# gue-ni/raytracer.c

Measured on AMD Instinct MI355X. Metric: ray-bounces/sec, higher is better.
Workload: dtype f64

## Files before the change

### include/rt_hip.h

```cpp
#ifndef RT_HIP_H
#define RT_HIP_H

#include <stddef.h>
#include <stdint.h>

#ifdef __cplusplus
extern "C" {
#endif

#define RT_HIP_TILE 8
#define RT_HIP_TILE_PIXELS 64

enum
{
  RT_HIP_OK = 0,
  RT_HIP_ENODEV = -1,
  RT_HIP_EINVAL = -2,
  RT_HIP_ENOMEM = -3,
  RT_HIP_ERUNTIME = -4,
  RT_HIP_ELIMIT = -5,
  RT_HIP_ECANCELLED = -6,
};

typedef struct
// ... 409 lines not shown
int rt_hip_selftest_math(int op, const double *h_a, const double *h_b, double *h_out, size_t n, int device);

int rt_hip_selftest_intersect(int kind, const double *h_rays, const double *h_prims, size_t n, double near_R,
                              uint8_t *h_hit, double *h_tuv, uint64_t *h_keep, int device);

enum
{
  RT_HIP_FAIL_ALLOC_PARK_WS = 1,
  RT_HIP_FAIL_ALLOC_WIDE_PEND = 2,
  RT_HIP_FAIL_ALLOC_TAIL_WS = 4
};
void rt_hip_selftest_fail_alloc(uint32_t mask);

uint64_t rt_hip_mixed_grid_launches(void);

int rt_hip_selftest_pool_slots(int device, uint32_t *park_slots_per_xcd, uint32_t *pend_slots_per_xcd);

int rt_hip_selftest_xcc(uint32_t n_workgroups, uint32_t h_counts[16], int device);


void rt_hip_set_cancel_flag(const volatile int *flag);

int rt_hip_render_image(const RtHipSphere *spheres, size_t n_spheres, const RtHipMesh *meshes,
                        size_t n_meshes, const RtHipCamera *camera, const RtHipParams *params,
                        int n_devices, float *h_image_rgb, uint8_t *h_image_rgb8, uint64_t *h_stats,
                        double *kernel_seconds);

void rt_hip_release_cache(void);
uint64_t rt_hip_cache_builds(void);

// ... 20 lines not shown
```

### raytracer.c_amd/csrc/pt_body_pooled.h

```cpp
#ifndef PT_BODY_POOLED_H
#define PT_BODY_POOLED_H


#ifndef PT_MIN_WAVES
#define PT_MIN_WAVES 5
#endif
#ifndef PT_MIN_WAVES_TRI
#define PT_MIN_WAVES_TRI 5
#endif
#ifndef PT_MIN_WAVES_CHK
#define PT_MIN_WAVES_CHK 5
#endif
#ifndef PT_MESH_BATCH
#define PT_MESH_BATCH 32
#endif
#ifndef PT_MESH_MAX_WAIT
#define PT_MESH_MAX_WAIT 16
#endif
#ifndef PT_DIR_PARK
#define PT_DIR_PARK 1
#endif
#ifndef PT_DIR_ROUNDS
#define PT_DIR_ROUNDS 4
#endif
// ... 2 lines not shown
#endif
#ifndef PT_DIR_MIN_LANES
#define PT_DIR_MIN_LANES 1
#endif
struct MixedUnit
{
  uint32_t j, chunk, chunks;
};
__device__ __forceinline__ MixedUnit mixed_unit(const PtLaunch &L, const bool LIST)
{
  const uint32_t n_whole = LIST ? 0u : L.n_whole;
  if (blockIdx.x < n_whole)
    return {blockIdx.x, 0u, 1u};
  const uint32_t r = blockIdx.x - n_whole, n_chunked = launch_slots(L, LIST) - n_whole;
  return {n_whole + r % n_chunked, r / n_chunked, L.sample_chunks};
}

template <bool CHECKER, bool TRIS, bool FILT_LDS, bool GEOM_LDS, bool REFR = false, bool MIXED = false>
__device__ __forceinline__ void render_tiles_pooled(const PtLaunch &L, const bool LIST)
{
  static_assert(!MIXED || !REFR, "the mixed grid: fixed-point sums only");
  static_assert(!REFR || (CHECKER && FILT_LDS && (GEOM_LDS || !TRIS)), "the pooled refraction kernels: sphere scenes (staged, or streamed from memory) and small staged mesh scenes, every material");
  extern __shared__ __attribute__((aligned(16))) double lds[];
  __shared__ float out_f[PT_TILE_PIXELS * 3];
  __shared__ uint8_t out_b[PT_TILE_PIXELS * 3 + 64];
  __shared__ unsigned long long wg_stats[2];
  __shared__ double cam_lds[PT_CAM_LDS_DOUBLES];
  __shared__ unsigned long long pix_sum[REFR ? 1 : PT_TILE_PIXELS * 3];
  __shared__ unsigned long long pix_win[REFR ? PT_TILE_PIXELS * 3 * PT_WIN_N : 1];
  __shared__ unsigned long long pend_free[REFR ? PT_BLOCK / 64 : 1][2];
// ... 51 lines not shown
  if (threadIdx.x < 3)
    pix_nan[threadIdx.x] = 0;
  if (!REFR && threadIdx.x < PT_TILE_PIXELS * 3)
    pix_sum[threadIdx.x] = 0;
  if (REFR)
  {
    for (uint32_t k = threadIdx.x; k < PT_TILE_PIXELS * 3 * PT_WIN_N; k += PT_BLOCK)
      pix_win[k] = 0;
    if (threadIdx.x < 2 * (PT_BLOCK / 64))
      pend_free[threadIdx.x >> 1][threadIdx.x & 1u] = ~0ull;
    if (threadIdx.x == 0)
      pend_slot_lds = pt_pool_acquire(L.pend_flags, L.pend_slots_per_xcd, L.status, PT_FAIL_PEND_SLOT);
  }
  if (threadIdx.x < PT_TILE_PIXELS)
  {
    const uint32_t t0 = L.tile_first + launch_slot(L, MIXED ? mixed_unit(L, LIST).j : blockIdx.x % launch_slots(L, LIST), LIST) * L.tile_stride;
    const uint32_t kx = (t0 % L.tiles_x) * PT_TILE + (threadIdx.x & 7u), ky = (t0 / L.tiles_x) * PT_TILE + (threadIdx.x >> 3);
    pix_key[threadIdx.x] = rt_rng_pixel_key(L.seed, ky * (uint32_t)L.width + kx);
  }
  camera_to_lds(L, cam_lds);
  PHASE(9);
  __syncthreads();
  PHASE(10);

  const uint32_t wave = threadIdx.x >> 6;
  const uint32_t slot = launch_slot(L, MIXED ? mixed_unit(L, LIST).j : blockIdx.x % launch_slots(L, LIST), LIST);
  const uint32_t chunk = MIXED ? mixed_unit(L, LIST).chunk : blockIdx.x / launch_slots(L, LIST);
  const uint32_t tile = L.tile_first + slot * L.tile_stride;
  const bool cull_ok = S.n_sph + S.n_tri <= 64u * CULL_WORDS;
  if (mf_sized && threadIdx.x < PT_MFMA16_ROWS)
  {
    uint16_t row[16];
    if (!pt_mfma16_row(L.scene.entry_src + PT_ENTRY_SRC_STRIDE * (size_t)(mf_first + threadIdx.x), L.near_R, S.filt_shift, row))
      atomicOr(&mf_bad, 1u);
    const uint32_t m = mfma16_row_of(threadIdx.x);
#pragma unroll
    for (int h = 0; h < 2; h++)
      mf_a[32 * h + m] = u32x4_t{row[8 * h + 0] | ((uint32_t)row[8 * h + 1] << 16), row[8 * h + 2] | ((uint32_t)row[8 * h + 3] << 16),
                                 row[8 * h + 4] | ((uint32_t)row[8 * h + 5] << 16), row[8 * h + 6] | ((uint32_t)row[8 * h + 7] << 16)};
  }
  if (SWAP && FILT_LDS && cull_ok)
// ... 449 lines not shown
    }
    PHASE(4);
    if (!PARK)
      radiance_to_sums();
    P.Ls = {0, 0, 0};
    PHASE(5);
  }

  if (n_rays)
  {
    atomicAdd(&wg_stats[0], (unsigned long long)n_rays);
    atomicAdd(&wg_stats[1], (unsigned long long)n_casts);
  }
  __syncthreads();
  PHASE(12);

  if (REFR)
  {
    if (!pend_ok && threadIdx.x < 3)
      pix_nan[threadIdx.x] = ~0ull;
    __syncthreads();
    if (L.sample_chunks == 1 && !L.acc_keep)
    {
      if (threadIdx.x < PT_TILE_PIXELS * 3)
      {
        const uint32_t t = threadIdx.x / 3u, c = threadIdx.x - 3u * t;
        const bool inside = (tile % L.tiles_x) * PT_TILE + (t & 7u) < (uint32_t)L.width && (tile / L.tiles_x) * PT_TILE + (t >> 3) < (uint32_t)L.height;
        win_normalize(&pix_win[threadIdx.x * PT_WIN_N]);
        double mean = win_value(&pix_win[threadIdx.x * PT_WIN_N]) * (1.0 / (double)L.samples);
        mean = ((pix_nan[c] >> t) & 1ull) ? __longlong_as_double(0x7FF8000000000000ll) : mean;
// ... 12 lines not shown
        unsigned long long *const acc = L.acc_ws + ((size_t)slot * (PT_TILE_PIXELS * 3) + threadIdx.x) * PT_WIN_N;
#pragma unroll
        for (int k = 0; k < PT_WIN_N; k++)
          if (w[k] != 0ull)
            atomicAdd(&acc[k], w[k]);
      }
      if (threadIdx.x < 3 && pix_nan[threadIdx.x] != 0)
        atomicOr(&L.acc_ws[(size_t)L.tile_count * (PT_TILE_PIXELS * 3 * PT_WIN_N) + (size_t)slot * 3 + threadIdx.x], pix_nan[threadIdx.x]);
      store_tile(L, out_f, out_b, wg_stats, tile, slot, S.n_sph + S.n_tri, false, chunk == 0);
    }
    if (pend_ok && threadIdx.x == 0)
      atomicExch(&L.pend_flags[pend_slot], 0u);
  }
  else if (MIXED ? ((!LIST && blockIdx.x < L.n_whole) || L.sample_chunks == 1) && !L.acc_keep : L.sample_chunks == 1 && !L.acc_keep)
  {
    finish_pixels(L, pix_sum, pix_nan, tile, out_f, out_b);
    __syncthreads();
    store_tile(L, out_f, out_b, wg_stats, tile, slot, S.n_sph + S.n_tri, true, true);
    PHASE(13);
#ifdef PT_PHASE
    if ((threadIdx.x & 63u) == 0u && L.stats && (blockIdx.x & 31u) == 0u)
      for (int k = 0; k < PT_PHASE_SLOTS; k++)
        atomicAdd(&L.stats[64 + k], pt_phase_acc[threadIdx.x >> 6][k]);
#endif
  }
  else
  {
    const uint32_t n_whole = MIXED && !LIST ? L.n_whole : 0u;
    if (threadIdx.x < PT_TILE_PIXELS * 3 && pix_sum[threadIdx.x] != 0)
      atomicAdd(&L.acc_ws[(size_t)(slot - n_whole) * (PT_TILE_PIXELS * 3) + threadIdx.x], pix_sum[threadIdx.x]);
    if (threadIdx.x < 3 && pix_nan[threadIdx.x] != 0)
      atomicOr(&L.acc_ws[(size_t)(L.tile_count - n_whole) * (PT_TILE_PIXELS * 3) + (size_t)(slot - n_whole) * 3 + threadIdx.x], pix_nan[threadIdx.x]);
    store_tile(L, out_f, out_b, wg_stats, tile, slot, S.n_sph + S.n_tri, false, chunk == 0);
  }
#ifdef PT_PHASE
  if (threadIdx.x == 0 && L.stats && (L.diag_flags & 4u))
  {
    L.stats[80 + 2 * (size_t)blockIdx.x] = wg_began;
    L.stats[81 + 2 * (size_t)blockIdx.x] = wall_clock64();
  }
#endif
}

#endif
```

### raytracer.c_amd/csrc/pt_device.h

```cpp
#ifndef PT_DEVICE_H
#define PT_DEVICE_H

#include <math.h>
#include <stdint.h>

#define PT_TILE 8
#define PT_TILE_PIXELS 64
#define PT_SLICES 4
#define PT_BLOCK 256
#define PT_MAT_STRIDE 8
#define PT_FILT_LDS_MAX 256
#ifndef PT_BVH_LEAF
#define PT_BVH_LEAF 15
#endif
#define PT_BVH_NODE_WORDS 16
#define PT_BVH_SRC_DOUBLES 16
#ifndef PT_BVH_COUNT_BITS
#define PT_BVH_COUNT_BITS 4
#endif
#define PT_BVH_LEAF_FLAG 0x80000000u
#define PT_BVH_STACK 24
#define PT_GEOM_STRIDE 4
#define PT_FILT_STRIDE 6
#define PT_TRI32_STRIDE 16
// ... 258 lines not shown
  char *park_ws;
  uint32_t *park_flags;
  uint32_t park_slots_per_xcd;
  double *pend_ws;
  uint32_t *pend_flags;
  uint32_t pend_slots_per_xcd, pend_entries;
  uint64_t pend_slot_doubles;
  uint32_t *status;
  unsigned long long *acc_ws;
  float *tiles_rgb;
  uint8_t *tiles_rgb8;
  unsigned long long *stats;
  const uint32_t *slot_list;
  uint32_t slot_count;
  uint32_t n_whole;
};

struct PtAovOut
{
  float *albedo, *normal, *depth;
  uint32_t *object, *hits;
};

struct PtQuery
{
  const double *rays;
  const double *t_max;
  uint64_t n;
  uint32_t camera_uv, normalize;
  uint32_t *status;
// ... 128 lines not shown
};
struct PtPlan
{
  int kernel;
  uint32_t sample_chunks;
  bool mixed;
  bool windowed;
  bool queued;
  uint32_t pend_entries, pend_columns;
};
PtPlan pt_plan_launch(const PtSceneView &scene, const PtPlanAsk &ask);
hipError_t pt_launch_render(const PtLaunch &launch, hipStream_t stream, int which);
bool pt_kernel_takes_chunks(int which);
uint32_t pt_resident_workgroups(int which, const PtSceneView &scene);
hipError_t pt_launch_resolve(const PtLaunch &launch, const uint32_t *tile_samples, hipStream_t stream, int which);
hipError_t pt_launch_tile_error(const float *cur, const float *prev, int width, int height, uint32_t tile_first, uint32_t tile_stride,
                                uint32_t tile_count, float *error, hipStream_t stream);
hipError_t pt_launch_tile_freeze(const float *error, double threshold, int dilate, uint8_t *keep, uint32_t *tile_samples, int width,
                                 int height, uint32_t tile_first, uint32_t tile_stride, uint32_t tile_count, uint32_t done,
                                 uint32_t *slot_list, uint32_t *live_count, hipStream_t stream);
static inline uint32_t pt_pend_entries(const PtSceneView &scene, uint32_t integrator, int32_t max_depth)
{
  const bool two_children = integrator == 1u ? scene.any_mirror_glass != 0u : scene.any_refract != 0u;
  return two_children ? (uint32_t)max_depth + 2u : 1u;
}
const char *pt_kernel_name_of(int which);
int pt_kernel_count(void);
unsigned long long pt_kernel_launches(int which);
uint32_t pt_pool_slots_per_xcd(bool park_pool);
#ifdef PT_DEV_KERNELS
// ... 111 lines not shown
```

### raytracer.c_amd/csrc/pt_kernel.hip

```cpp
#include <hip/hip_runtime.h>
#include <stdint.h>
#include <stdlib.h>
#include <atomic>

#include "pt_device.h"
#include "rt_rng.h"

#include "pt_math.h"
#include "pt_intersect.h"
#include "pt_filter.h"
#include "pt_scene_ctx.h"
#include "pt_trace.h"
#include "pt_body_pooled.h"
#include "pt_body_queued.h"
#include "pt_body_static.h"

enum PtKernelProps : uint32_t
{
  PEND_POOL = 1u, QUEUED = 2u, STAGES_NONE = 4u, WIDE_PEND = 8u, CHUNKS = 16u, WINDOWED = 32u, MIXED = 64u
};

#ifndef PT_MIN_WAVES_QUEUED
#define PT_MIN_WAVES_QUEUED 4
#endif
// ... 493 lines not shown
    const bool inside = (tile % L.tiles_x) * PT_TILE + (t & 7u) < (uint32_t)L.width &&
                        (tile / L.tiles_x) * PT_TILE + (t >> 3) < (uint32_t)L.height;
    const double inv_s = 1.0 / (double)samples;
    double mean = ((double)(long long)sums[threadIdx.x] * L.acc_inv_scale) * inv_s;
    const double quiet_nan = __longlong_as_double(0x7FF8000000000000ll);
    mean = ((nan_mask[c] >> t) & 1ull) ? quiet_nan : mean;
    out_f[threadIdx.x] = inside ? (float)mean : 0.f;
    out_b[threadIdx.x] = inside ? tonemap(mean) : 0;
  }
}

extern "C" __global__ __launch_bounds__(PT_BLOCK) void pt_resolve_tiles(const PtLaunch L, const uint32_t *tile_samples)
{
  __shared__ float out_f[PT_TILE_PIXELS * 3];
  __shared__ uint8_t out_b[PT_TILE_PIXELS * 3 + 64];
  const uint32_t slot = L.n_whole + blockIdx.x;
  const int32_t samples = resolve_samples(L, tile_samples, slot);
  const uint32_t tile = L.tile_first + slot * L.tile_stride;
  if (L.acc_windows)
  {
    if (threadIdx.x < PT_TILE_PIXELS * 3)
    {
      const uint32_t t = threadIdx.x / 3u, c = threadIdx.x - 3u * t;
      const bool inside = (tile % L.tiles_x) * PT_TILE + (t & 7u) < (uint32_t)L.width && (tile / L.tiles_x) * PT_TILE + (t >> 3) < (uint32_t)L.height;
      unsigned long long w[PT_WIN_N];
#pragma unroll
      for (int k = 0; k < PT_WIN_N; k++)
        w[k] = L.acc_ws[((size_t)slot * (PT_TILE_PIXELS * 3) + threadIdx.x) * PT_WIN_N + k];
      win_normalize(w);
      double mean = win_value(w) * (1.0 / (double)samples);
      const unsigned long long nan_mask = L.acc_ws[(size_t)L.tile_count * (PT_TILE_PIXELS * 3 * PT_WIN_N) + (size_t)slot * 3 + c];
// ... 112 lines not shown
  part[threadIdx.x] = n;
  __syncthreads();
  for (uint32_t step = 1; step < PT_COMPACT_THREADS; step <<= 1)
  {
    const uint32_t add = threadIdx.x >= step ? part[threadIdx.x - step] : 0u;
    __syncthreads();
    part[threadIdx.x] += add;
    __syncthreads();
  }
  uint32_t at = part[threadIdx.x] - n;
  for (uint32_t k = k0; k < k1; k++)
    if (tile_samples[k] == 0u)
      slot_list[at++] = k;
  if (threadIdx.x == PT_COMPACT_THREADS - 1)
    *live_count = part[threadIdx.x];
}

extern "C" __global__ __launch_bounds__(256) void pt_selftest_math(int op, const double *a, const double *b,
                                                                  double *out, size_t n)
{
  __shared__ double tab[PT_ATAN_TAB];
  atan_table_to_lds(tab);
  __syncthreads();
  for (size_t i = (size_t)blockIdx.x * blockDim.x + threadIdx.x; i < n; i += (size_t)gridDim.x * blockDim.x)
  {
    double r = 0;
    if (op == 0)
      r = sqrt_unscaled(a[i]);
    else if (op == 1)
      r = div_small_int(a[i], b[i], 1.0 / b[i]);
// ... 580 lines not shown
  if (k.has(PEND_POOL) && (launch.pend_ws == nullptr || launch.pend_entries < pt_pend_entries(launch.scene, launch.integrator, launch.max_depth) ||
                      launch.pend_slot_doubles < (uint64_t)launch.pend_entries * PT_PEND_FIELDS_HOST * k.pend_columns()))
    return hipErrorInvalidValue;
  const bool queued = k.has(QUEUED);
  if (queued && (launch.park_ws == nullptr || launch.park_slots_per_xcd == 0u))
    return hipErrorInvalidValue;
  if (launch.sample_chunks > 1 && !k.has(CHUNKS))
    return hipErrorInvalidValue;
  if (queued)
    lds_bytes += (k.has(STAGES_NONE) ? (size_t)0 : (size_t)pt_filt_pair_slots(launch.scene.n_spheres) * 8u) +
                 (((size_t)max(launch.scene.bvh_depth, 1u) * PT_BLOCK * 3u + 15u) & ~(size_t)15u);
  if (launch.acc_keep && (k.has(CHUNKS) ? launch.acc_ws == nullptr || (launch.acc_windows != 0u) != k.has(WINDOWED) : launch.slice_ws == nullptr))
    return hipErrorInvalidValue;
  if (launch.n_whole != 0u && (!k.has(MIXED) || launch.n_whole >= launch.tile_count || launch.sample_chunks < 2u || launch.acc_keep || launch.slot_list))
    return hipErrorInvalidValue;
  const uint32_t n_chunked = launch.tile_count - launch.n_whole;
  if (launch.sample_chunks > 1 && !launch.acc_keep)
  {
    if ((launch.acc_windows != 0u) != k.has(WINDOWED) || launch.acc_ws == nullptr)
      return hipErrorInvalidValue;
    hipError_t e = hipMemsetAsync(launch.acc_ws, 0, (size_t)n_chunked * (k.has(WINDOWED) ? PT_ACC_WS_WORDS_WIN : PT_ACC_WS_WORDS) * sizeof(unsigned long long), stream);
    if (e != hipSuccess)
      return e;
  }
  if ((launch.slot_list != nullptr) != (launch.slot_count != 0u) || (launch.slot_list && !launch.acc_keep) || launch.slot_count > launch.tile_count)
    return hipErrorInvalidValue;
  const uint32_t n_units = launch.n_whole + (launch.slot_list ? launch.slot_count : n_chunked) * launch.sample_chunks;
  hipError_t e = launch_staged(kernel, queued ? (n_units + PT_BLOCK / 64 - 1) / (PT_BLOCK / 64) : n_units, lds_bytes, stream, launch);
  if (e == hipSuccess && launch.sample_chunks > 1 && !launch.acc_keep)
    e = launch_staged(pt_resolve_tiles, n_chunked, 0, stream, launch, static_cast<const uint32_t *>(nullptr));
// ... 45 lines not shown
  const uint32_t tiles_x = ((uint32_t)width + PT_TILE - 1) / PT_TILE, waves = PT_BLOCK / 64u;
  hipLaunchKernelGGL(pt_tile_error, dim3((tile_count + waves - 1u) / waves), dim3(PT_BLOCK), 0, stream, cur, prev, width, height, tiles_x,
                     tile_first, tile_stride, tile_count, error);
  return hipGetLastError();
}

hipError_t pt_launch_tile_freeze(const float *error, double threshold, int dilate, uint8_t *keep, uint32_t *tile_samples, int width,
                                 int height, uint32_t tile_first, uint32_t tile_stride, uint32_t tile_count, uint32_t done,
                                 uint32_t *slot_list, uint32_t *live_count, hipStream_t stream)
{
  const uint32_t tiles_x = ((uint32_t)width + PT_TILE - 1) / PT_TILE, tiles_y = ((uint32_t)height + PT_TILE - 1) / PT_TILE;
  if (error)
    hipLaunchKernelGGL(pt_tile_keep, dim3((tile_count + 255u) / 256u), dim3(256), 0, stream, error, tile_samples, tiles_x, tiles_y, tile_first,
                       tile_stride, tile_count, threshold, dilate, keep);
  hipLaunchKernelGGL(pt_tile_compact, dim3(1), dim3(PT_COMPACT_THREADS), 0, stream, keep, tile_samples, tile_count, done, slot_list, live_count);
  return hipGetLastError();
}

hipError_t pt_launch_selftest_intersect(int kind, const double *rays, const double *prims, const double *entry_src,
                                        float *filt, float *tri32, uint32_t n, double near_R, double filt_shift,
                                        uint8_t *hit, double *tuv, unsigned long long *keep, hipStream_t stream)
{
  if (n == 0)
    return hipSuccess;
  if (kind == 2 && (!PT_MFMA16 || n % 64u != 0u))
    return hipErrorNotSupported;
  hipLaunchKernelGGL(pt_build_filter, dim3(min(1024u, (n + 255u) / 256u)), dim3(256), 0, stream, entry_src, n, near_R, filt);
  if (kind == 2)
  {
    hipLaunchKernelGGL(pt_selftest_mfma16, dim3(n / 64u), dim3(64), 0, stream, rays, prims, entry_src, reinterpret_cast<const f32x2 *>(filt), n,
// ... 111 lines not shown
```

### raytracer.c_amd/csrc/rt_hip_shim.hip

```cpp
#include <hip/hip_runtime.h>
#include <rccl/rccl.h>

#include <algorithm>
#include <atomic>
#include <chrono>
#include <cmath>
#include <cstdarg>
#include <cstddef>
#include <cstdio>
#include <cstdlib>
#include <cstring>
#include <limits>
#include <mutex>
#include <new>
#include <utility>
#include <vector>

#include "pt_device.h"
#include "rt_hip.h"
#include "rt_rng.h"
#include "bvh_build.h"
#include "rt_staging.h"

static_assert(sizeof(RtHipSphere) == 88, "RtHipSphere must match the reference Object");
// ... 231 lines not shown

}

struct TableSet
{
  double near_R = 0;
  float *filt = nullptr, *bvh_nodes = nullptr;
  hipEvent_t built = nullptr;
  std::vector<std::pair<hipStream_t, hipEvent_t>> readers;
  uint64_t stamp = 0;
  int users = 0;
  bool owned = false;
};
#define RT_TABLE_SETS 8

struct RtHipScene
{
  int device = 0;
  PtSceneView view{};
  mutable std::mutex table_mutex;
  mutable std::vector<TableSet> tables;
  mutable uint64_t table_clock = 0;
  size_t filt_bytes = 0, bvh_nodes_bytes = 0;
  mutable char *park_ws = nullptr;
  mutable uint32_t park_slots_per_xcd = 0;
  mutable bool park_tried = false;
  void *blob = nullptr;
  double reach = 0;
  double max_emission = 0;
  bool any_mirror_glass = false;
  double max_center = 0;
  int n_big = 0;
  double big_r[8] = {0}, big_c[8] = {0};
// ... 74 lines not shown
  m[2] = color[1] * inv;
  m[3] = color[2] * inv;
  m[4] = emission[0];
  m[5] = emission[1];
  m[6] = emission[2];
  uint64_t bits = flags;
  memcpy(&m[7], &bits, sizeof bits);
}




std::atomic<uint32_t> g_fail_alloc{0};

thread_local int g_last_kernel = -1;

size_t pad256(size_t b) { return (b + 255) & ~(size_t)255; }

hipError_t table_set_wait(const TableSet &t)
{
  hipError_t first = t.built ? hipEventSynchronize(t.built) : hipSuccess;
  for (auto &r : t.readers)
    if (const hipError_t e = hipEventSynchronize(r.second); first == hipSuccess)
      first = e;
  return first;
}

void table_set_free(TableSet &t)
{
  for (auto &r : t.readers)
// ... 30 lines not shown
    for (const TableSet &t : scene->tables)
      if (t.users > 0)
        return fail(RT_HIP_EINVAL, "a launch of this scene is being submitted");
    return RT_HIP_OK;
  }
  int drain() const
  {
    for (const TableSet &t : scene->tables)
      HIP_TRY(table_set_wait(t));
    return RT_HIP_OK;
  }
  void stale() const
  {
    for (TableSet &t : scene->tables)
      t.near_R = -1.0;
  }
  int broke(hipError_t e, const char *what) const
  {
    (void)hipGetLastError();
    scene->unusable = true;
    return fail(RT_HIP_ERUNTIME, "%s: %s; the scene is unusable now (destroy it)", what, hipGetErrorString(e));
  }
};

int acquire_tables(const RtHipScene *scene, double near_R, hipStream_t stream, float **filt, float **bvh_nodes, size_t *slot)
{
  std::lock_guard<std::mutex> lock(scene->table_mutex);
  std::vector<TableSet> &tables = scene->tables;
  if (const int rc = scene_usable(scene, "a launch"))
    return rc;
// ... 349 lines not shown
    }
  {
    std::lock_guard<std::mutex> slock(g_status_mutex);
    for (int d = 0; d < 64; d++)
      if (g_status[d])
      {
        (void)hipSetDevice(d);
        (void)hipDeviceSynchronize();
        (void)hipFree(g_status[d]);
        g_status[d] = nullptr;
      }
  }
  (void)hipSetDevice(prev);
}

struct GridTailWs
{
  unsigned long long *ws = nullptr;
  size_t bytes = 0;
  hipEvent_t done = nullptr;
  hipStream_t stream = nullptr;
  bool used = false;
  uint32_t resident = 0;
  int resident_kernel = -1;
  size_t resident_lds = 0;
};
std::mutex g_tail_mutex;
GridTailWs g_tail[64];
std::atomic<uint64_t> g_mixed_launches{0};

constexpr uint32_t GRID_TAIL_MIN_ROUNDS = 8, GRID_TAIL_ROUNDS = 1, GRID_TAIL_CHUNKS = 4, GRID_TAIL_MIN_SAMPLES = 128;

bool grid_split_for(const PtLaunch &L, const PtPlan &plan, int device, uint32_t *n_whole, uint32_t *chunks)
{
  if (!plan.mixed || plan.sample_chunks != 1u || L.acc_keep || L.slot_list || L.tile_count < 2u || L.samples < 2)
    return false;
  const char *uni = getenv("RT_HIP_GRID_UNIFORM");
  if (uni && uni[0] == '1')
    return false;
  if (const char *e = getenv("RT_HIP_GRID_SPLIT"))
// ... 17 lines not shown
    if (t.resident_kernel != plan.kernel || t.resident_lds != lds)
    {
      t.resident = pt_resident_workgroups(plan.kernel, L.scene);
      t.resident_kernel = plan.kernel;
      t.resident_lds = lds;
    }
    resident = t.resident;
  }
  if (resident == 0u || (uint64_t)L.tile_count < (uint64_t)GRID_TAIL_MIN_ROUNDS * resident)
    return false;
  *n_whole = L.tile_count - GRID_TAIL_ROUNDS * resident;
  *chunks = GRID_TAIL_CHUNKS;
  return true;
}

unsigned long long *grid_tail_ws(int device, uint32_t n_chunked, hipStream_t stream)
{
  if (device < 0 || device >= 64 || (g_fail_alloc.load() & RT_HIP_FAIL_ALLOC_TAIL_WS))
    return nullptr;
  GridTailWs &t = g_tail[device];
  const size_t need = (size_t)n_chunked * PT_ACC_WS_WORDS * sizeof(unsigned long long);
  if (t.bytes < need)
  {
    if (t.ws)
    {
      if (hipDeviceSynchronize() != hipSuccess)
      {
        (void)hipGetLastError();
        return nullptr;
      }
      (void)hipFree(t.ws);
      t.ws = nullptr;
    }
    t.bytes = 0;
    t.used = false;
    if (hipMalloc(&t.ws, need) != hipSuccess)
    {
      (void)hipGetLastError();
      t.ws = nullptr;
      return nullptr;
    }
    t.bytes = need;
  }
  if (!t.done && hipEventCreateWithFlags(&t.done, hipEventDisableTiming) != hipSuccess)
  {
    (void)hipGetLastError();
    t.done = nullptr;
    return nullptr;
  }
  if (t.used && t.stream != stream && hipStreamWaitEvent(stream, t.done, 0) != hipSuccess)
  {
    (void)hipGetLastError();
    return nullptr;
  }
  return t.ws;
}

void grid_tail_used(int device, hipStream_t stream)
{
  GridTailWs &t = g_tail[device];
  if (hipEventRecord(t.done, stream) != hipSuccess)
  {
    (void)hipGetLastError();
    (void)hipStreamSynchronize(stream);
    t.used = false;
    return;
  }
  t.stream = stream;
  t.used = true;
}

void grid_tail_release()
{
  std::lock_guard<std::mutex> lock(g_tail_mutex);
  int prev = 0;
  (void)hipGetDevice(&prev);
  for (int d = 0; d < 64; d++)
    if (g_tail[d].ws || g_tail[d].done)
    {
      (void)hipSetDevice(d);
      (void)hipDeviceSynchronize();
      if (g_tail[d].done)
        (void)hipEventDestroy(g_tail[d].done);
      if (g_tail[d].ws)
        (void)hipFree(g_tail[d].ws);
      g_tail[d] = GridTailWs();
    }
  (void)hipSetDevice(prev);
}

uint32_t tiles_x_of(int width) { return ((uint32_t)width + PT_TILE - 1) / PT_TILE; }
uint32_t tiles_y_of(int height) { return ((uint32_t)height + PT_TILE - 1) / PT_TILE; }

int check_params(const RtHipParams *p)
{
  if (!p)
    return fail(RT_HIP_EINVAL, "params is NULL");
  if (p->width < 2 || p->height < 2)
    return fail(RT_HIP_EINVAL, "width and height must be >= 2 (the reference divides by width-1, height-1)");
  if (p->samples < 1 || p->samples > (1 << 26))
// ... 3237 lines not shown
  v.n_bvh_nodes = c->n_triangles ? std::max(1u, c->n_triangles / 8u) : 0u;
  v.any_checker = c->any_checker ? 1u : 0u;
  v.any_refract = c->any_refract ? 1u : 0u;
  v.any_mirror_glass = c->any_mirror_glass ? 1u : 0u;
  v.wide_range = c->wide_range ? 1u : 0u;
  v.mesh_round = c->mesh_round ? 1u : 0u;
  const PtPlanAsk ask = {.integrator = c->integrator, .samples = c->samples_per_chunk, .max_depth = c->max_depth, .max_emission = c->max_emission,
                         .sample_chunks = 1, .have_park_ws = c->have_park_ws != 0, .wide_pend_ok = c->wide_pend_ok != 0};
  return pt_kernel_name_of(pt_plan_launch(v, ask).kernel);
}

void rt_hip_selftest_fail_alloc(uint32_t mask) { g_fail_alloc.store(mask); }

uint64_t rt_hip_mixed_grid_launches(void) { return g_mixed_launches.load(); }

int rt_hip_selftest_pool_slots(int device, uint32_t *park_slots_per_xcd, uint32_t *pend_slots_per_xcd)
{
  if (!have_device(device))
    return fail(RT_HIP_ENODEV, "no HIP device %d", device);
  DeviceScope scope(device);
  HIP_TRY(scope.status);
  if (park_slots_per_xcd)
    *park_slots_per_xcd = pt_pool_slots_per_xcd(true);
  if (pend_slots_per_xcd)
    *pend_slots_per_xcd = pt_pool_slots_per_xcd(false);
  return RT_HIP_OK;
}

int rt_hip_pool_bytes(int device, size_t *park_ws_bytes, size_t *pend_pool_bytes)
{
// ... 126 lines not shown
      rc = fail(RT_HIP_EINVAL, "tile_count x sample_chunks exceeds the grid limit");
    std::unique_lock<std::mutex> tail_lock(g_tail_mutex, std::defer_lock);
    uint32_t n_whole = 0, tail_chunks = 0;
    if (!rc && sample_chunks == 1 && !d_workspace && grid_split_for(L, plan, scene->device, &n_whole, &tail_chunks))
    {
      tail_lock.lock();
      if (unsigned long long *ws = grid_tail_ws(scene->device, L.tile_count - n_whole, st))
      {
        L.acc_ws = ws;
        L.n_whole = n_whole;
        L.sample_chunks = tail_chunks;
      }
      else
        tail_lock.unlock();
    }
    const hipError_t e = rc ? hipSuccess : pt_launch_render(L, st, plan.kernel);
    if (tail_lock.owns_lock())
    {
      grid_tail_used(scene->device, st);
      if (e == hipSuccess && L.n_whole != 0u)
        g_mixed_launches.fetch_add(1);
      tail_lock.unlock();
    }
    if (pend_lock.owns_lock())
      pend_lock.unlock();
    release_tables(scene, slot, st);
    if (!rc)
      rc = launched(e, pt_kernel_name_of(plan.kernel));
    if (!rc)
      g_last_kernel = plan.kernel;
    return rc;
  });
}


int rt_hip_accum_create(const RtHipScene *scene, const RtHipCamera *camera, const RtHipParams *params, RtHipAccum **out)
{
  if (out)
    *out = nullptr;
  if (!scene || !camera || !params || !out)
    return fail(RT_HIP_EINVAL, "scene, camera, params and out are required");
  if (params->samples < 1)
    return fail(RT_HIP_EINVAL, "the sample budget (params->samples) must be >= 1");
  return guarded("rt_hip_accum_create", [&]() -> int {
    PtLaunch L;
// ... 1031 lines not shown
```

### raytracer.c_amd/rt_amd/abi.py

```python
import ctypes as C
import os

PKG_DIR = os.path.dirname(os.path.dirname(os.path.abspath(__file__)))
REPO_ROOT = os.path.dirname(PKG_DIR)
SHIM_PATH = os.environ.get("RT_HIP_SHIM_PATH") or os.path.join(PKG_DIR, "csrc", "librt_hip.so")
HOST_PATH = os.path.join(PKG_DIR, "host", "libraytracer_amd.so")

M_DEFAULT, M_REFLECTION, M_REFRACTION, M_CHECKERED = 2, 4, 8, 16
TILE, TILE_PIXELS, TILE_FLOATS = 8, 64, 192
STAT_RAYS, STAT_CASTS, STAT_TESTS, STAT_SAMPLES, NSTATS = 0, 1, 2, 3, 4
FAIL_ALLOC_PARK_WS, FAIL_ALLOC_WIDE_PEND, FAIL_ALLOC_TAIL_WS = 1, 2, 4
FAIL_PEND_SLOT, FAIL_PARK_SLOT = 1, 2
EINVAL = -2
PASS_FN = C.CFUNCTYPE(None, C.c_int, C.c_int, C.c_double, C.c_void_p)


class Vec2(C.Structure):
    _fields_ = [("x", C.c_double), ("y", C.c_double)]


class Vec3(C.Structure):
    _fields_ = [("x", C.c_double), ("y", C.c_double), ("z", C.c_double)]

    def tuple(self):
# ... 229 lines not shown
    "rt_hip_untile": (C.c_int, [C.c_void_p, C.c_void_p, C.c_int32, C.c_int32, C.c_uint32, C.c_uint32, C.c_uint32,
                                C.c_void_p, C.c_void_p, C.c_void_p]),
    "rt_hip_set_cancel_flag": (None, [C.c_void_p]),
    "rt_hip_release_cache": (None, []),
    "rt_hip_cache_builds": (C.c_uint64, []),
    "rt_hip_set_device_map": (C.c_int, [C.POINTER(C.c_int), C.c_int]),
    "rt_hip_last_image_phases": (None, [C.POINTER(C.c_double)]),
    "rt_hip_pool_bytes": (C.c_int, [C.c_int, C.POINTER(C.c_size_t), C.POINTER(C.c_size_t)]),
    "rt_hip_last_launch_kernel": (C.c_char_p, []),
    "rt_hip_kernel_count": (C.c_int, []),
    "rt_hip_kernel_launches": (C.c_char_p, [C.c_int, C.POINTER(C.c_uint64)]),
    "rt_hip_kernel_for_class": (C.c_char_p, [C.c_void_p]),
    "rt_hip_launch_status": (C.c_int, [C.c_int, C.POINTER(C.c_uint32)]),
    "rt_hip_selftest_fail_alloc": (None, [C.c_uint32]),
    "rt_hip_mixed_grid_launches": (C.c_uint64, []),
    "rt_hip_selftest_pool_slots": (C.c_int, [C.c_int, C.POINTER(C.c_uint32), C.POINTER(C.c_uint32)]),
    "rt_hip_render_aov_tiles": (C.c_int, [C.c_void_p, C.POINTER(Camera), C.POINTER(RtHipParams), C.POINTER(RtHipAov), C.c_void_p]),
    "rt_hip_untile_aov": (C.c_int, [C.POINTER(RtHipAov), C.c_int32, C.c_int32, C.c_uint32, C.c_uint32, C.c_uint32,
                                    C.POINTER(RtHipAov), C.c_void_p]),
    "rt_hip_render_aov_image": (C.c_int, [C.POINTER(Object), C.c_size_t, C.POINTER(RtHipMesh), C.c_size_t, C.POINTER(Camera),
                                          C.POINTER(RtHipParams), C.c_int, C.POINTER(RtHipAov)]),
    "rt_hip_aov_kernel_name": (C.c_char_p, [C.c_void_p]),
    "rt_hip_aov_kernel_count": (C.c_int, []),
    "rt_hip_aov_kernel_launches": (C.c_char_p, [C.c_int, C.POINTER(C.c_uint64)]),
    "rt_hip_query_defaults": (None, [C.POINTER(RtHipQueryParams)]),
    "rt_hip_query_rays": (C.c_int, [C.c_void_p, C.c_void_p, C.c_void_p, C.c_uint64, C.POINTER(RtHipQueryParams), C.POINTER(RtHipHits),
                                    C.c_void_p]),
    "rt_hip_query_rays_host": (C.c_int, [C.POINTER(Object), C.c_size_t, C.POINTER(RtHipMesh), C.c_size_t, C.c_void_p, C.c_void_p,
                                         C.c_uint64, C.POINTER(RtHipQueryParams), C.c_int, C.POINTER(RtHipHits)]),
    "rt_hip_query_kernel_name": (C.c_char_p, [C.c_void_p]),
# ... 273 lines not shown
```

Measured before the change: 51.50 billion.

## Schedule mixed-grid tiles by measured per-tile cost from the previous frame

Records per-tile ray counts during mixed-grid launches and sorts tiles by cost with a single-workgroup bucket sort kernel. On the next launch with a matching scene and parameter key, workgroups take tiles in descending-cost order so expensive tiles start first, which shrinks the tail imbalance. It adds a cost atomic per workgroup, an extra order kernel per launch, and indirection through an order table, and it only applies after a first frame has populated the table.

Result: no change. 51.61 billion (median of 6 runs) (+0.2%).

```diff
diff --git a/include/rt_hip.h b/include/rt_hip.h
--- a/include/rt_hip.h
+++ b/include/rt_hip.h
@@ -447,6 +447,15 @@
 
 uint64_t rt_hip_mixed_grid_launches(void);
 
+enum
+{
+  RT_HIP_TILE_ORDER_NONE = 0,
+  RT_HIP_TILE_ORDER_TABLE = 1,
+  RT_HIP_TILE_ORDER_REVERSED = 2
+};
+int rt_hip_last_launch_tile_order(void);
+int rt_hip_selftest_tile_order(int device, const uint32_t *cost, uint32_t n, int reverse, uint32_t *order);
+
 int rt_hip_selftest_pool_slots(int device, uint32_t *park_slots_per_xcd, uint32_t *pend_slots_per_xcd);
 
 int rt_hip_selftest_xcc(uint32_t n_workgroups, uint32_t h_counts[16], int device);
diff --git a/raytracer.c_amd/csrc/pt_body_pooled.h b/raytracer.c_amd/csrc/pt_body_pooled.h
--- a/raytracer.c_amd/csrc/pt_body_pooled.h
+++ b/raytracer.c_amd/csrc/pt_body_pooled.h
@@ -40,6 +40,10 @@
     return {blockIdx.x, 0u, 1u};
   const uint32_t r = blockIdx.x - n_whole, n_chunked = launch_slots(L, LIST) - n_whole;
   return {n_whole + r % n_chunked, r / n_chunked, L.sample_chunks};
+}
+__device__ __forceinline__ uint32_t mixed_slot(const PtLaunch &L, uint32_t j, const bool LIST)
+{
+  return !LIST && L.tile_order ? L.tile_order[j] : launch_slot(L, j, LIST);
 }
 
 template <bool CHECKER, bool TRIS, bool FILT_LDS, bool GEOM_LDS, bool REFR = false, bool MIXED = false>
@@ -121,7 +125,7 @@
   }
   if (threadIdx.x < PT_TILE_PIXELS)
   {
-    const uint32_t t0 = L.tile_first + launch_slot(L, MIXED ? mixed_unit(L, LIST).j : blockIdx.x % launch_slots(L, LIST), LIST) * L.tile_stride;
+    const uint32_t t0 = L.tile_first + (MIXED ? mixed_slot(L, mixed_unit(L, LIST).j, LIST) : launch_slot(L, blockIdx.x % launch_slots(L, LIST), LIST)) * L.tile_stride;
     const uint32_t kx = (t0 % L.tiles_x) * PT_TILE + (threadIdx.x & 7u), ky = (t0 / L.tiles_x) * PT_TILE + (threadIdx.x >> 3);
     pix_key[threadIdx.x] = rt_rng_pixel_key(L.seed, ky * (uint32_t)L.width + kx);
   }
@@ -131,7 +135,7 @@
   PHASE(10);
 
   const uint32_t wave = threadIdx.x >> 6;
-  const uint32_t slot = launch_slot(L, MIXED ? mixed_unit(L, LIST).j : blockIdx.x % launch_slots(L, LIST), LIST);
+  const uint32_t slot = MIXED ? mixed_slot(L, mixed_unit(L, LIST).j, LIST) : launch_slot(L, blockIdx.x % launch_slots(L, LIST), LIST);
   const uint32_t chunk = MIXED ? mixed_unit(L, LIST).chunk : blockIdx.x / launch_slots(L, LIST);
   const uint32_t tile = L.tile_first + slot * L.tile_stride;
   const bool cull_ok = S.n_sph + S.n_tri <= 64u * CULL_WORDS;
@@ -611,6 +615,11 @@
   }
   __syncthreads();
   PHASE(12);
+  uint32_t entry_e = MIXED ? mixed_unit(L, LIST).j : 0u;
+  if (MIXED)
+    asm volatile("" : "+s"(entry_e));
+  const uint32_t slot_e = MIXED && !LIST && L.tile_order ? L.tile_order[entry_e] : slot;
+  const uint32_t tile_e = MIXED ? L.tile_first + slot_e * L.tile_stride : tile;
 
   if (REFR)
   {
@@ -653,9 +662,9 @@
   }
   else if (MIXED ? ((!LIST && blockIdx.x < L.n_whole) || L.sample_chunks == 1) && !L.acc_keep : L.sample_chunks == 1 && !L.acc_keep)
   {
-    finish_pixels(L, pix_sum, pix_nan, tile, out_f, out_b);
+    finish_pixels(L, pix_sum, pix_nan, tile_e, out_f, out_b);
     __syncthreads();
-    store_tile(L, out_f, out_b, wg_stats, tile, slot, S.n_sph + S.n_tri, true, true);
+    store_tile(L, out_f, out_b, wg_stats, tile_e, slot_e, S.n_sph + S.n_tri, true, true);
     PHASE(13);
 #ifdef PT_PHASE
     if ((threadIdx.x & 63u) == 0u && L.stats && (blockIdx.x & 31u) == 0u)
@@ -666,12 +675,15 @@
   else
   {
     const uint32_t n_whole = MIXED && !LIST ? L.n_whole : 0u;
+    const uint32_t rec = (MIXED && !LIST && L.tile_order ? mixed_unit(L, LIST).j : slot_e) - n_whole;
     if (threadIdx.x < PT_TILE_PIXELS * 3 && pix_sum[threadIdx.x] != 0)
-      atomicAdd(&L.acc_ws[(size_t)(slot - n_whole) * (PT_TILE_PIXELS * 3) + threadIdx.x], pix_sum[threadIdx.x]);
+      atomicAdd(&L.acc_ws[(size_t)rec * (PT_TILE_PIXELS * 3) + threadIdx.x], pix_sum[threadIdx.x]);
     if (threadIdx.x < 3 && pix_nan[threadIdx.x] != 0)
-      atomicOr(&L.acc_ws[(size_t)(L.tile_count - n_whole) * (PT_TILE_PIXELS * 3) + (size_t)(slot - n_whole) * 3 + threadIdx.x], pix_nan[threadIdx.x]);
-    store_tile(L, out_f, out_b, wg_stats, tile, slot, S.n_sph + S.n_tri, false, chunk == 0);
-  }
+      atomicOr(&L.acc_ws[(size_t)(L.tile_count - n_whole) * (PT_TILE_PIXELS * 3) + (size_t)rec * 3 + threadIdx.x], pix_nan[threadIdx.x]);
+    store_tile(L, out_f, out_b, wg_stats, tile_e, slot_e, S.n_sph + S.n_tri, false, chunk == 0);
+  }
+  if (MIXED && !LIST && L.tile_cost && threadIdx.x == 128)
+    atomicAdd(&L.tile_cost[slot_e], (uint32_t)(wg_stats[0] >> 6));
 #ifdef PT_PHASE
   if (threadIdx.x == 0 && L.stats && (L.diag_flags & 4u))
   {
diff --git a/raytracer.c_amd/csrc/pt_device.h b/raytracer.c_amd/csrc/pt_device.h
--- a/raytracer.c_amd/csrc/pt_device.h
+++ b/raytracer.c_amd/csrc/pt_device.h
@@ -296,6 +296,8 @@
   const uint32_t *slot_list;
   uint32_t slot_count;
   uint32_t n_whole;
+  const uint32_t *tile_order;
+  uint32_t *tile_cost;
 };
 
 struct PtAovOut
@@ -454,6 +456,7 @@
 bool pt_kernel_takes_chunks(int which);
 uint32_t pt_resident_workgroups(int which, const PtSceneView &scene);
 hipError_t pt_launch_resolve(const PtLaunch &launch, const uint32_t *tile_samples, hipStream_t stream, int which);
+hipError_t pt_launch_tile_order(const uint32_t *cost, uint32_t n, bool reverse, uint32_t *order, hipStream_t stream);
 hipError_t pt_launch_tile_error(const float *cur, const float *prev, int width, int height, uint32_t tile_first, uint32_t tile_stride,
                                 uint32_t tile_count, float *error, hipStream_t stream);
 hipError_t pt_launch_tile_freeze(const float *error, double threshold, int dilate, uint8_t *keep, uint32_t *tile_samples, int width,
diff --git a/raytracer.c_amd/csrc/pt_kernel.hip b/raytracer.c_amd/csrc/pt_kernel.hip
--- a/raytracer.c_amd/csrc/pt_kernel.hip
+++ b/raytracer.c_amd/csrc/pt_kernel.hip
@@ -531,7 +531,7 @@
 {
   __shared__ float out_f[PT_TILE_PIXELS * 3];
   __shared__ uint8_t out_b[PT_TILE_PIXELS * 3 + 64];
-  const uint32_t slot = L.n_whole + blockIdx.x;
+  const uint32_t slot = L.tile_order ? L.tile_order[L.n_whole + blockIdx.x] : L.n_whole + blockIdx.x;
   const int32_t samples = resolve_samples(L, tile_samples, slot);
   const uint32_t tile = L.tile_first + slot * L.tile_stride;
   if (L.acc_windows)
@@ -674,6 +674,95 @@
       slot_list[at++] = k;
   if (threadIdx.x == PT_COMPACT_THREADS - 1)
     *live_count = part[threadIdx.x];
+}
+
+#define PT_ORDER_THREADS 1024u
+#define PT_ORDER_BUCKETS 512u
+__device__ __forceinline__ uint32_t tile_order_bucket(uint32_t cost, uint32_t top)
+{
+  return top ? (PT_ORDER_BUCKETS - 1u) - (uint32_t)((uint64_t)cost * (PT_ORDER_BUCKETS - 1u) / top) : 0u;
+}
+extern "C" __global__ __launch_bounds__(PT_ORDER_THREADS) void pt_tile_order(const uint32_t *__restrict__ cost, uint32_t n, uint32_t reverse,
+                                                                           uint32_t *__restrict__ order)
+{
+  constexpr uint32_t WAVES = PT_ORDER_THREADS / 64u;
+  __shared__ uint32_t at[WAVES][PT_ORDER_BUCKETS];
+  __shared__ uint32_t start[PT_ORDER_BUCKETS];
+  __shared__ uint32_t max_cost;
+  const uint32_t lane = threadIdx.x & 63u, wave = threadIdx.x >> 6;
+  for (uint32_t k = threadIdx.x; k < WAVES * PT_ORDER_BUCKETS; k += PT_ORDER_THREADS)
+    (&at[0][0])[k] = 0u;
+  if (threadIdx.x == 0)
+    max_cost = 0u;
+  __syncthreads();
+  uint32_t m = 0u;
+  for (uint32_t i = threadIdx.x; i < n; i += PT_ORDER_THREADS)
+    m = max(m, cost[i]);
+  atomicMax(&max_cost, m);
+  __syncthreads();
+  const uint32_t top = max_cost;
+  const uint32_t per = (uint32_t)(((uint64_t)n + PT_ORDER_THREADS - 1u) / PT_ORDER_THREADS) * 64u;
+  const uint32_t k0 = (uint32_t)min((uint64_t)n, (uint64_t)wave * per), k1 = (uint32_t)min((uint64_t)n, (uint64_t)k0 + per);
+  for (uint32_t i = k0 + lane; i < k1; i += 64u)
+    atomicAdd(&at[wave][tile_order_bucket(cost[i], top)], 1u);
+  __syncthreads();
+  if (threadIdx.x < PT_ORDER_BUCKETS)
+  {
+    uint32_t t = 0u;
+    for (uint32_t w = 0; w < WAVES; w++)
+    {
+      const uint32_t c = at[w][threadIdx.x];
+      at[w][threadIdx.x] = t;
+      t += c;
+    }
+    start[threadIdx.x] = t;
+  }
+  __syncthreads();
+  if (wave == 0u)
+  {
+    constexpr uint32_t PER_LANE = PT_ORDER_BUCKETS / 64u;
+    uint32_t v[PER_LANE], s = 0u;
+#pragma unroll
+    for (uint32_t k = 0; k < PER_LANE; k++)
+    {
+      v[k] = start[lane * PER_LANE + k];
+      s += v[k];
+    }
+    uint32_t inc = s;
+    for (uint32_t d = 1; d < 64u; d <<= 1)
+    {
+      const uint32_t below = __shfl_up(inc, d);
+      inc += lane >= d ? below : 0u;
+    }
+    uint32_t run = inc - s;
+#pragma unroll
+    for (uint32_t k = 0; k < PER_LANE; k++)
+    {
+      start[lane * PER_LANE + k] = run;
+      run += v[k];
+    }
+  }
+  __syncthreads();
+  for (uint32_t i0 = k0; i0 < k1; i0 += 64u)
+  {
+    const uint32_t i = i0 + lane;
+    const bool have = i < k1;
+    const uint32_t b = have ? tile_order_bucket(cost[i], top) : 0xFFFFFFFFu;
+    uint32_t below = 0u, same = 0u;
+#pragma unroll
+    for (uint32_t j = 0; j < 64u; j++)
+    {
+      const bool eq = (uint32_t)__builtin_amdgcn_readlane((int)b, (int)j) == b;
+      same += eq ? 1u : 0u;
+      below += eq && j < lane ? 1u : 0u;
+    }
+    const uint32_t rank = have ? start[b] + at[wave][b] + below : n;
+    if (rank < n)
+      order[reverse ? n - 1u - rank : rank] = i;
+    __builtin_amdgcn_wave_barrier();
+    if (have && below == 0u)
+      at[wave][b] += same;
+  }
 }
 
 extern "C" __global__ __launch_bounds__(256) void pt_selftest_math(int op, const double *a, const double *b,
@@ -1284,6 +1373,8 @@
     return hipErrorInvalidValue;
   if (launch.n_whole != 0u && (!k.has(MIXED) || launch.n_whole >= launch.tile_count || launch.sample_chunks < 2u || launch.acc_keep || launch.slot_list))
     return hipErrorInvalidValue;
+  if ((launch.tile_order || launch.tile_cost) && (!k.has(MIXED) || launch.acc_keep || launch.slot_list))
+    return hipErrorInvalidValue;
   const uint32_t n_chunked = launch.tile_count - launch.n_whole;
   if (launch.sample_chunks > 1 && !launch.acc_keep)
   {
@@ -1359,6 +1450,14 @@
     hipLaunchKernelGGL(pt_tile_keep, dim3((tile_count + 255u) / 256u), dim3(256), 0, stream, error, tile_samples, tiles_x, tiles_y, tile_first,
                        tile_stride, tile_count, threshold, dilate, keep);
   hipLaunchKernelGGL(pt_tile_compact, dim3(1), dim3(PT_COMPACT_THREADS), 0, stream, keep, tile_samples, tile_count, done, slot_list, live_count);
+  return hipGetLastError();
+}
+
+hipError_t pt_launch_tile_order(const uint32_t *cost, uint32_t n, bool reverse, uint32_t *order, hipStream_t stream)
+{
+  if (!cost || !order || n == 0u || n > 0x7FFFFFFFu)
+    return hipErrorInvalidValue;
+  hipLaunchKernelGGL(pt_tile_order, dim3(1), dim3(PT_ORDER_THREADS), 0, stream, cost, n, reverse ? 1u : 0u, order);
   return hipGetLastError();
 }
 
diff --git a/raytracer.c_amd/csrc/rt_hip_shim.hip b/raytracer.c_amd/csrc/rt_hip_shim.hip
--- a/raytracer.c_amd/csrc/rt_hip_shim.hip
+++ b/raytracer.c_amd/csrc/rt_hip_shim.hip
@@ -269,9 +269,13 @@
 };
 #define RT_TABLE_SETS 8
 
+std::atomic<uint64_t> g_scene_uids{0};
+
 struct RtHipScene
 {
   int device = 0;
+  const uint64_t uid = g_scene_uids.fetch_add(1) + 1;
+  uint64_t generation = 0;
   PtSceneView view{};
   mutable std::mutex table_mutex;
   mutable std::vector<TableSet> tables;
@@ -376,6 +380,7 @@
 std::atomic<uint32_t> g_fail_alloc{0};
 
 thread_local int g_last_kernel = -1;
+thread_local int g_last_tile_order = RT_HIP_TILE_ORDER_NONE;
 
 size_t pad256(size_t b) { return (b + 255) & ~(size_t)255; }
 
@@ -436,6 +441,7 @@
   {
     for (TableSet &t : scene->tables)
       t.near_R = -1.0;
+    scene->generation++;
   }
   int broke(hipError_t e, const char *what) const
   {
@@ -815,6 +821,20 @@
   (void)hipSetDevice(prev);
 }
 
+struct TileOrderKey
+{
+  uint64_t scene_uid = 0, generation = 0;
+  int32_t width = 0, height = 0, samples = 0, max_depth = 0;
+  uint32_t integrator = 0, tile_first = 0, tile_stride = 0, tile_count = 0;
+  int kernel = -1;
+  bool operator==(const TileOrderKey &o) const
+  {
+    return scene_uid == o.scene_uid && generation == o.generation && width == o.width && height == o.height && samples == o.samples &&
+           max_depth == o.max_depth && integrator == o.integrator && tile_first == o.tile_first && tile_stride == o.tile_stride &&
+           tile_count == o.tile_count && kernel == o.kernel;
+  }
+};
+
 struct GridTailWs
 {
   unsigned long long *ws = nullptr;
@@ -825,6 +845,10 @@
   uint32_t resident = 0;
   int resident_kernel = -1;
   size_t resident_lds = 0;
+  uint32_t *tab = nullptr;
+  size_t tab_tiles = 0;
+  bool order_valid = false;
+  TileOrderKey order_key;
 };
 std::mutex g_tail_mutex;
 GridTailWs g_tail[64];
@@ -872,6 +896,22 @@
   return true;
 }
 
+bool grid_tail_join(GridTailWs &t, hipStream_t stream)
+{
+  if (!t.done && hipEventCreateWithFlags(&t.done, hipEventDisableTiming) != hipSuccess)
+  {
+    (void)hipGetLastError();
+    t.done = nullptr;
+    return false;
+  }
+  if (t.used && t.stream != stream && hipStreamWaitEvent(stream, t.done, 0) != hipSuccess)
+  {
+    (void)hipGetLastError();
+    return false;
+  }
+  return true;
+}
+
 unsigned long long *grid_tail_ws(int device, uint32_t n_chunked, hipStream_t stream)
 {
   if (device < 0 || device >= 64 || (g_fail_alloc.load() & RT_HIP_FAIL_ALLOC_TAIL_WS))
@@ -900,18 +940,45 @@
     }
     t.bytes = need;
   }
-  if (!t.done && hipEventCreateWithFlags(&t.done, hipEventDisableTiming) != hipSuccess)
-  {
-    (void)hipGetLastError();
-    t.done = nullptr;
+  return grid_tail_join(t, stream) ? t.ws : nullptr;
+}
+
+int tile_order_mode()
+{
+  const char *e = getenv("RT_HIP_TILE_ORDER");
+  if (!e || !e[0])
+    return 1;
+  return e[0] == '0' ? 0 : (strcmp(e, "reverse") == 0 ? 3 : 2);
+}
+
+uint32_t *tile_order_tab(int device, uint32_t n_tiles, hipStream_t stream)
+{
+  if (device < 0 || device >= 64)
     return nullptr;
-  }
-  if (t.used && t.stream != stream && hipStreamWaitEvent(stream, t.done, 0) != hipSuccess)
-  {
-    (void)hipGetLastError();
-    return nullptr;
-  }
-  return t.ws;
+  GridTailWs &t = g_tail[device];
+  if (t.tab_tiles < n_tiles)
+  {
+    if (t.tab)
+    {
+      if (hipDeviceSynchronize() != hipSuccess)
+      {
+        (void)hipGetLastError();
+        return nullptr;
+      }
+      (void)hipFree(t.tab);
+      t.tab = nullptr;
+    }
+    t.tab_tiles = 0;
+    t.order_valid = false;
+    if (hipMalloc(&t.tab, (size_t)n_tiles * 2u * sizeof(uint32_t)) != hipSuccess)
+    {
+      (void)hipGetLastError();
+      t.tab = nullptr;
+      return nullptr;
+    }
+    t.tab_tiles = n_tiles;
+  }
+  return grid_tail_join(t, stream) ? t.tab : nullptr;
 }
 
 void grid_tail_used(int device, hipStream_t stream)
@@ -934,7 +1001,7 @@
   int prev = 0;
   (void)hipGetDevice(&prev);
   for (int d = 0; d < 64; d++)
-    if (g_tail[d].ws || g_tail[d].done)
+    if (g_tail[d].ws || g_tail[d].done || g_tail[d].tab)
     {
       (void)hipSetDevice(d);
       (void)hipDeviceSynchronize();
@@ -942,6 +1009,8 @@
         (void)hipEventDestroy(g_tail[d].done);
       if (g_tail[d].ws)
         (void)hipFree(g_tail[d].ws);
+      if (g_tail[d].tab)
+        (void)hipFree(g_tail[d].tab);
       g_tail[d] = GridTailWs();
     }
   (void)hipSetDevice(prev);
@@ -4209,6 +4278,29 @@
 
 uint64_t rt_hip_mixed_grid_launches(void) { return g_mixed_launches.load(); }
 
+int rt_hip_last_launch_tile_order(void) { return g_last_tile_order; }
+
+int rt_hip_selftest_tile_order(int device, const uint32_t *cost, uint32_t n, int reverse, uint32_t *order)
+{
+  if (!cost || !order || n == 0u || n > 0x7FFFFFFFu)
+    return fail(RT_HIP_EINVAL, "cost, order and 1 .. 2^31 - 1 tiles are required");
+  if (!have_device(device))
+    return fail(RT_HIP_ENODEV, "no HIP device %d", device);
+  return guarded("rt_hip_selftest_tile_order", [&]() -> int {
+    DeviceScope scope(device);
+    HIP_TRY(scope.status);
+    DeviceBuffer tab;
+    HIP_TRY(tab.alloc((size_t)n * 2u * sizeof(uint32_t)));
+    uint32_t *const d = tab.at<uint32_t>();
+    HIP_TRY(hipMemcpy(d, cost, (size_t)n * sizeof(uint32_t), hipMemcpyHostToDevice));
+    HIP_TRY(hipMemset(d + n, 0xFF, (size_t)n * sizeof(uint32_t)));
+    if (const int rc = launched(pt_launch_tile_order(d, n, reverse != 0, d + n, nullptr), "pt_tile_order"))
+      return rc;
+    HIP_TRY(hipMemcpy(order, d + n, (size_t)n * sizeof(uint32_t), hipMemcpyDeviceToHost));
+    return RT_HIP_OK;
+  });
+}
+
 int rt_hip_selftest_pool_slots(int device, uint32_t *park_slots_per_xcd, uint32_t *pend_slots_per_xcd)
 {
   if (!have_device(device))
@@ -4365,7 +4457,41 @@
       else
         tail_lock.unlock();
     }
-    const hipError_t e = rc ? hipSuccess : pt_launch_render(L, st, plan.kernel);
+    const int order_mode = tile_order_mode();
+    int order_used = RT_HIP_TILE_ORDER_NONE;
+    GridTailWs &tail = g_tail[scene->device >= 0 && scene->device < 64 ? scene->device : 0];
+    const TileOrderKey order_key = {scene->uid, scene->generation, L.width, L.height, L.samples, L.max_depth, L.integrator,
+                                    L.tile_first, L.tile_stride, L.tile_count, plan.kernel};
+    if (!rc && sample_chunks == 1 && !d_workspace && plan.mixed && plan.sample_chunks == 1u && !L.acc_keep && !L.slot_list && L.tile_count >= 2u &&
+        (order_mode >= 2 || (order_mode == 1 && L.n_whole != 0u)))
+    {
+      if (!tail_lock.owns_lock())
+        tail_lock.lock();
+      uint32_t *const tab = tile_order_tab(scene->device, L.tile_count, st);
+      if (tab && hipMemsetAsync(tab, 0, (size_t)L.tile_count * sizeof(uint32_t), st) == hipSuccess)
+      {
+        L.tile_cost = tab;
+        if (tail.order_valid && tail.order_key == order_key)
+        {
+          L.tile_order = tab + tail.tab_tiles;
+          order_used = order_mode == 3 ? RT_HIP_TILE_ORDER_REVERSED : RT_HIP_TILE_ORDER_TABLE;
+        }
+      }
+      else
+      {
+        (void)hipGetLastError();
+        if (L.n_whole == 0u)
+          tail_lock.unlock();
+      }
+    }
+    hipError_t e = rc ? hipSuccess : pt_launch_render(L, st, plan.kernel);
+    if (L.tile_cost)
+    {
+      tail.order_valid = e == hipSuccess && pt_launch_tile_order(L.tile_cost, L.tile_count, order_mode == 3, L.tile_cost + tail.tab_tiles, st) == hipSuccess;
+      tail.order_key = order_key;
+      if (e == hipSuccess && !tail.order_valid)
+        (void)hipGetLastError();
+    }
     if (tail_lock.owns_lock())
     {
       grid_tail_used(scene->device, st);
@@ -4379,7 +4505,10 @@
     if (!rc)
       rc = launched(e, pt_kernel_name_of(plan.kernel));
     if (!rc)
+    {
       g_last_kernel = plan.kernel;
+      g_last_tile_order = order_used;
+    }
     return rc;
   });
 }
diff --git a/raytracer.c_amd/rt_amd/abi.py b/raytracer.c_amd/rt_amd/abi.py
--- a/raytracer.c_amd/rt_amd/abi.py
+++ b/raytracer.c_amd/rt_amd/abi.py
@@ -267,6 +267,8 @@
     "rt_hip_launch_status": (C.c_int, [C.c_int, C.POINTER(C.c_uint32)]),
     "rt_hip_selftest_fail_alloc": (None, [C.c_uint32]),
     "rt_hip_mixed_grid_launches": (C.c_uint64, []),
+    "rt_hip_last_launch_tile_order": (C.c_int, []),
+    "rt_hip_selftest_tile_order": (C.c_int, [C.c_int, C.POINTER(C.c_uint32), C.c_uint32, C.c_int, C.POINTER(C.c_uint32)]),
     "rt_hip_selftest_pool_slots": (C.c_int, [C.c_int, C.POINTER(C.c_uint32), C.POINTER(C.c_uint32)]),
     "rt_hip_render_aov_tiles": (C.c_int, [C.c_void_p, C.POINTER(Camera), C.POINTER(RtHipParams), C.POINTER(RtHipAov), C.c_void_p]),
     "rt_hip_untile_aov": (C.c_int, [C.POINTER(RtHipAov), C.c_int32, C.c_int32, C.c_uint32, C.c_uint32, C.c_uint32,
```
